# TimeEscaper/distributed_eigenspaces

Measured on AMD Instinct MI355X. Metric: samples/sec ingested + time-to-eigenspace (d=8192,k=64) at 1/8 GPU; sinθ error, higher is better.
Workload: dtype f32

## Files before the change

distributed_eigenspaces_amd/csrc/capi.hip:

```cpp
#include <stdarg.h>
#include <stdio.h>
#include <string.h>

#include <atomic>
#include <vector>

#include "deig_internal.hpp"

namespace deig {

static thread_local char g_err[1024] = "";

const char* last_error() { return g_err; }

void set_error(const char* fmt, ...) {
  va_list ap;
  va_start(ap, fmt);
  vsnprintf(g_err, sizeof(g_err), fmt, ap);
  va_end(ap);
}

int fail(int code, const char* fmt, ...) {
  va_list ap;
  va_start(ap, fmt);
// ... 10 lines not shown
    return 256;
  }
  int v = cache[dev].load(std::memory_order_relaxed);
  if (!v) {
    if (hipDeviceGetAttribute(&v, hipDeviceAttributeMultiprocessorCount, dev) != hipSuccess ||
        v <= 0) {
      (void)hipGetLastError();
      v = 256;
    }
    cache[dev].store(v, std::memory_order_relaxed);
  }
  return v;
}

}

using namespace deig;

extern "C" {

int deig_version(void) { return 0x000600; }

void deig_shutdown(void) {
  if (status_pool_empty()) return;
  (void)hipDeviceSynchronize();
  status_pool_drain();
  (void)hipGetLastError();
}

const char* deig_last_error(void) { return g_err; }

void deig_solver_opts_init(deig_solver_opts* o) {
  if (!o) return;
  memset(o, 0, sizeof(*o));
  o->size = (int)sizeof(deig_solver_opts);
  o->sweep_algo = DEIG_SWEEP_AUTO;
  o->rr_every = 0;
  o->chebyshev = 1;
  o->cheb_above = -1.f;
  o->deflate = 1;
  o->deflate_early = 1;
  o->jacobi_early_sweeps = -1;
  o->jacobi_early_above = -1.f;
  o->fast_until = 1e-3f;
  o->round_until = 1e-4f;
  o->debug = 0;
  o->half_until = 1e-2f;
}

// ... 46 lines not shown
  if (algo != DEIG_SYRK_AUTO) return algo;
  return n >= DEIG_SYRK_SPLIT_MIN_ROWS ? DEIG_SYRK_SPLIT3 : DEIG_SYRK_FP32;
}

size_t deig_syrk_workspace_ex(int64_t n, int64_t d, int algo) {
  algo = syrk_resolve(n, algo & ~DEIG_SYRK_ACCUMULATE);
  if (algo == DEIG_SYRK_FP32) return syrk_workspace_bytes(n, d);
  if (algo == DEIG_SYRK_SPLIT3) return syrk_split_workspace_bytes(n, d);
  return 0;
}

int deig_syrk_f32_ex(const float* X, int64_t n, int64_t d, int64_t ldx, float alpha, float* S,
                     int64_t lds, int algo, void* ws, size_t ws_bytes, void* stream) {
  g_err[0] = 0;
  const bool acc = (algo & DEIG_SYRK_ACCUMULATE) != 0;
  algo = syrk_resolve(n, algo & ~DEIG_SYRK_ACCUMULATE);
  if (acc && algo != DEIG_SYRK_SPLIT3)
    return fail(DEIG_EINVAL, "syrk: DEIG_SYRK_ACCUMULATE needs the split3 algorithm");
  if (algo == DEIG_SYRK_FP32)
    return syrk_launch(X, n, d, ldx, alpha, S, lds, ws, ws_bytes, (hipStream_t)stream);
  if (algo == DEIG_SYRK_SPLIT3)
    return syrk_split_launch(X, n, d, ldx, alpha, S, lds, ws, ws_bytes, (hipStream_t)stream, acc);
  return fail(DEIG_EINVAL, "syrk: unknown algorithm %d", algo);
}

size_t deig_syrk_workspace(int64_t n, int64_t d) {
  return deig_syrk_workspace_ex(n, d, DEIG_SYRK_DEFAULT);
}

int deig_syrk_f32(const float* X, int64_t n, int64_t d, int64_t ldx, float alpha, float* S,
                  int64_t lds, void* ws, size_t ws_bytes, void* stream) {
  return deig_syrk_f32_ex(X, n, d, ldx, alpha, S, lds, DEIG_SYRK_DEFAULT, ws, ws_bytes, stream);
}

size_t deig_syrk_bf16_workspace(int64_t n, int64_t d) { return syrk_bf16_workspace_bytes(n, d); }

int deig_syrk_bf16(const void* X, int64_t n, int64_t d, int64_t ldx, float alpha, float* S,
                   int64_t lds, int flags, void* ws, size_t ws_bytes, void* stream) {
  g_err[0] = 0;
  return syrk_bf16_launch(X, n, d, ldx, alpha, S, lds, flags, ws, ws_bytes, (hipStream_t)stream);
}

size_t deig_syrk_shift_workspace(int64_t n, int64_t d, int xtype) {
  return syrk_shift_workspace_bytes(n, d, xtype);
}

// ... 465 lines not shown
```

distributed_eigenspaces_amd/csrc/deig_internal.hpp:

```cpp
#pragma once

#include <hip/hip_runtime.h>
#include <stdint.h>
#include <stddef.h>

#include "../../include/deig.h"

namespace deig {

typedef float f32x16 __attribute__((ext_vector_type(16)));
typedef float f32x4 __attribute__((ext_vector_type(4)));
typedef float f32x2 __attribute__((ext_vector_type(2)));
typedef double f64x2 __attribute__((ext_vector_type(2)));
typedef __attribute__((address_space(3))) void lds_void;

void set_error(const char* fmt, ...);
int fail(int code, const char* fmt, ...);
const char* last_error();

#define DEIG_HIP_CHECK(expr)                                                          \
  do {                                                                                \
    hipError_t e__ = (expr);                                                          \
    if (e__ != hipSuccess)                                                            \
      return ::deig::fail(DEIG_EHIP, "%s:%d %s: %s", __FILE__, __LINE__, #expr,       \
// ... 30 lines not shown

struct Carve {
  char* base;
  size_t cap;
  size_t off = 0;
  Carve(void* b, size_t c) : base(static_cast<char*>(b)), cap(c) {}
  template <class T>
  T* take(size_t count) {
    off = align_up(off, 256);
    T* p = reinterpret_cast<T*>(base ? base + off : nullptr);
    off += count * sizeof(T);
    return p;
  }
  bool ok() const { return off <= cap; }
};

size_t syrk_workspace_bytes(int64_t n, int64_t d);
int syrk_launch(const float* X, int64_t n, int64_t d, int64_t ldx, float alpha, float* S,
                int64_t lds, void* ws, size_t ws_bytes, hipStream_t stream);
size_t syrk_split_workspace_bytes(int64_t n, int64_t d);
int syrk_split_launch(const float* X, int64_t n, int64_t d, int64_t ldx, float alpha, float* S,
                      int64_t lds, void* ws, size_t ws_bytes, hipStream_t stream,
                      bool accumulate = false);

size_t syrk_bf16_workspace_bytes(int64_t n, int64_t d);
int syrk_bf16_launch(const void* X, int64_t n, int64_t d, int64_t ldx, float alpha, float* S,
                     int64_t lds, int flags, void* ws, size_t ws_bytes, hipStream_t stream);

size_t syrk_shift_workspace_bytes(int64_t n, int64_t d, int xtype);
int syrk_shift_launch(const void* X, int xtype, int64_t n, int64_t d, int64_t ldx, double alpha,
                      double* S64, int64_t lds64, float* S, int64_t lds, void* ws, size_t ws_bytes,
                      hipStream_t stream);

size_t syrk_centered_workspace_bytes(int64_t n, int64_t d, int xtype);
int syrk_centered_launch(const void* X, int xtype, int64_t n, int64_t d, int64_t ldx,
                         const double* center, double alpha, double* S64, int64_t lds64, float* S,
                         int64_t lds, double* mean_out, void* ws, size_t ws_bytes,
                         hipStream_t stream);
size_t colsum_workspace_bytes(int64_t n, int64_t d);
int colsum_launch(const void* X, int xtype, int64_t n, int64_t d, int64_t ldx, double* sums,
                  void* ws, size_t ws_bytes, hipStream_t stream);

size_t syrk_u8_workspace_bytes(int64_t n, int64_t d, int mode);
int syrk_u8_launch(const uint8_t* X, int64_t n, int64_t d, int64_t ldx, int mode, double alpha,
                   float* S, int64_t lds, double* S64, int64_t lds64, void* ws, size_t ws_bytes,
                   hipStream_t stream);
// ... 205 lines not shown
```

distributed_eigenspaces_amd/csrc/lds_dma.hpp:

```cpp
#pragma once

#include "deig_internal.hpp"

namespace deig {

typedef int i32x4 __attribute__((ext_vector_type(4)));

__device__ __forceinline__ i32x4 make_rsrc(const void* base, uint32_t nrec) {
  const uint64_t a = reinterpret_cast<uint64_t>(base);
  i32x4 r;
  r[0] = (int)(uint32_t)a;
  r[1] = (int)((uint32_t)(a >> 32) & 0xffffu);
  r[2] = (int)nrec;
  r[3] = 0x00020000;
  return r;
}

__device__ __forceinline__ void dma16(i32x4 rsrc, int voff, const void* lds_dst) {
  const unsigned m0v = (unsigned)(uintptr_t)(lds_void*)lds_dst;
  asm volatile("s_mov_b32 m0, %2\n\tbuffer_load_dwordx4 %0, %1, 0 offen lds"
               :
               : "v"(voff), "s"(rsrc), "s"(m0v)
               : "memory", "m0");
}

template <int N>
__device__ __forceinline__ void wait_vm() {
  asm volatile("s_waitcnt vmcnt(%0)" ::"n"(N) : "memory");
}

}
```

distributed_eigenspaces_amd/csrc/syrk_split.hip:

```cpp
#include <cmath>
#include <cstdlib>

#include "bf16_split.hpp"
#include "deig_internal.hpp"
#include "lds_dma.hpp"

namespace deig {
namespace {

constexpr int BT = 256;
constexpr int ROWS_PAD = 32;
constexpr int NTHR = 512;
constexpr int SLICE_B = BT * 16;
constexpr int SLAB = BT * BT;
constexpr int SPLIT_YB = 256;
constexpr int SUPER_H = 8, SUPER_W = 4;
constexpr int BLOCK_B = 8 * SLICE_B;
constexpr size_t DEFAULT_CHUNK_BYTES = size_t(64) << 30;

struct SSched {
  unsigned char* XP;
  float* S;
  float* part;
  float* accs;
  const int* order;
  int64_t lds, dp;
  int64_t NK;
  int nseg;
  int d, nt, T, G, q, R;
  float alpha;
  int beta;
  int flush_kt;
  unsigned* pace;
  int pace_kt;
  const float* X;
  int64_t ldx, nrows;
  float* corr;
};

constexpr int kChipPaceEvery = 2;
#ifdef DEIG_AB_SYRK_FLUSH_STAGGER
// ... 56 lines not shown
  const int items = s.R * s.nseg;
  return L < items ? (items - 1 - L) / s.G + 1 : 0;
}

__device__ __forceinline__ void rem_item(const SSched& s, int L, int u, int& tile, int& slot, int& sg) {
  const int i = L + u * s.G;
  sg = i / s.R;
  const int r = i - sg * s.R;
  tile = s.q * s.G + r;
  slot = sg * s.R + r;
}

struct WorkItem {
  int tile, slot, seg;
  int64_t k0, k1;
  bool partial;
  PaceSeq pc;
};

template <bool HALF>
__device__ __forceinline__ WorkItem work_item(const SSched& s, int L, int w) {
  WorkItem it{0, 0, 0, 0, s.NK, w >= s.q, PaceSeq{0, 0u, 0u}};
  const unsigned nx = xcd_blocks(s);
  const unsigned P = s.pace_kt > 0 ? (unsigned)(s.NK / s.pace_kt) : 0u;
  if (!it.partial) {
    it.tile = w * s.G + L;
    it.pc = PaceSeq{(int)P, (unsigned)w * P * nx, nx};
    if (HALF) {
      it.pc.g = true;
      it.pc.gbase = (unsigned)w * (P / kChipPaceEvery) * (unsigned)s.G;
      it.pc.gmult = (unsigned)s.G;
    }
    return it;
  }
  const int u = w - s.q;
  rem_item(s, L, u, it.tile, it.slot, it.seg);
  it.k0 = __builtin_amdgcn_readfirstlane((int)(s.NK * it.seg / s.nseg));
  it.k1 = __builtin_amdgcn_readfirstlane((int)(s.NK * (it.seg + 1) / s.nseg));
  const int Pm = (HALF && s.pace_kt > 0 && s.nseg > 0) ? (int)(s.NK / s.nseg / s.pace_kt) : 0;
  if (Pm > 0) {
    const int items = s.R * s.nseg;
    unsigned before = 0;
    unsigned gb = (unsigned)s.q * (P / kChipPaceEvery) * (unsigned)s.G;
    for (int v = 0; v < u; ++v) {
      before += (unsigned)rem_active(s, L, v);
      gb += (unsigned)min(s.G, items - v * s.G) * (unsigned)(Pm / kChipPaceEvery);
    }
    it.pc = PaceSeq{Pm, (unsigned)s.q * P * nx + before * (unsigned)Pm, (unsigned)rem_active(s, L, u)};
    it.pc.g = true;
    it.pc.gbase = gb;
    it.pc.gmult = (unsigned)min(s.G, items - u * s.G);
  }
  return it;
}

constexpr int PANEL_B = 8 * SLICE_B;
constexpr int BUF_B = 2 * PANEL_B;

constexpr int OCT_B = 2 * SLICE_B;

__device__ __forceinline__ void stage_x(const SSched& s, int64_t kt, int f0, unsigned char* buf,
                                        int wave, int voff) {
  const int64_t row0 = kt * 32 + 8 * (wave & 3);
  int64_t rv = s.nrows - row0;
// ... 170 lines not shown
  }
  if (!diag) {
#pragma unroll
    for (int u = 0; u < 4; ++u) s.S[(int64_t)(ib + u) * s.lds + j] = v[u];
    const f32x4 w = {v[0], v[1], v[2], v[3]};
    *reinterpret_cast<f32x4*>(s.S + (int64_t)j * s.lds + ib) = w;
  } else {
#pragma unroll
    for (int u = 0; u < 4; ++u)
      if (ib + u >= j) {
        s.S[(int64_t)(ib + u) * s.lds + j] = v[u];
        s.S[(int64_t)j * s.lds + ib + u] = v[u];
      }
  }
}

struct TileCtx {
  int lane, wave, wi, wj;
  int ti, tj, i0, j0;
  bool diag;
  float* slab;
};

__device__ __forceinline__ TileCtx tile_ctx(const SSched& s, const WorkItem& it) {
  TileCtx c;
  c.lane = threadIdx.x & 63;
  c.wave = __builtin_amdgcn_readfirstlane(threadIdx.x >> 6);
  c.wi = c.wave >> 2;
  c.wj = c.wave & 3;
  const int tt = __builtin_amdgcn_readfirstlane(s.order[it.tile]);
  c.ti = tt & 0xffff;
  c.tj = tt >> 16;
  c.i0 = c.ti * BT;
  c.j0 = c.tj * BT;
  c.diag = (c.ti == c.tj);
  c.slab = it.partial ? s.part + (int64_t)it.slot * SLAB : s.accs + (int64_t)blockIdx.x * SLAB;
  return c;
}

template <bool IDLE = false>
__device__ __forceinline__ void finish_tile(const SSched& s, const TileCtx c, Acc& acc, bool flushed,
                                            bool partial) {
  if constexpr (!IDLE)
    if (flushed) unflush(c.slab, acc, c.wave, c.lane);
  if (partial) {
#pragma unroll
    for (int q = 0; q < NQUAD; ++q)
      *slab_at(c.slab, c.wave, q, c.lane) = f32x4{acc.at(q, 0), acc.at(q, 1), acc.at(q, 2), acc.at(q, 3)};
    return;
  }
  if constexpr (IDLE) return;
#pragma unroll
  for (int q = 0; q < NQUAD; ++q) {
    const float a[4] = {acc.at(q, 0), acc.at(q, 1), acc.at(q, 2), acc.at(q, 3)};
    store4(s, c.i0 + 128 * c.wi + Acc::qrow(q, c.lane), c.j0 + 64 * c.wj + Acc::qcol(q, c.lane), c.diag, a);
  }
}

template <bool SQ>
__device__ __forceinline__ void segment(const SSched& s, unsigned char* lds, const WorkItem& it) {
  const TileCtx tc = tile_ctx(s, it);
  const int lane = tc.lane, wave = tc.wave, wi = tc.wi, wj = tc.wj;
  const int64_t k0 = it.k0;
  float* const slab = tc.slab;
  const int fx0 = (wave >= 4 && !tc.diag) ? tc.j0 : tc.i0;
  const int fv = s.d - fx0;
  const int xvoff = 4 * lane < fv ? lane * 16 : (1 << 30);
  float sq[4] = {0.f, 0.f, 0.f, 0.f};

  Acc acc;
  acc.zero();
  bool flushed = false;
  const int64_t nkt = it.k1 - k0;
  if (nkt > 0) {
    wait_vm<0>();
    __syncthreads();
    stage_x(s, k0, fx0, lds, wave, xvoff);
    wait_vm<0>();
    const int64_t rv0 = s.nrows - (k0 * 32 + 8 * (wave & 3));
    convert_x<SQ>(lds, wave, lane, rv0 < 0 ? 0 : rv0 > 8 ? 8 : (int)rv0, fv, sq);
    int cur = 0, nxt = 1, since = 0;
    PaceState pace(it.pc);
    for (int64_t t = 0; t < nkt; ++t) {
      pace_point(s, it.pc, pace);
// ... 14 lines not shown
        flushed = true;
        since = 0;
      }
      cur = cur + 1 == 2 ? 0 : cur + 1;
      nxt = nxt + 1 == 2 ? 0 : nxt + 1;
    }
  }
  if (SQ) {
    float* c = s.corr + (int64_t)(it.seg * 4 + wave) * s.dp + tc.i0;
#pragma unroll
    for (int h = 0; h < 2; ++h)
      *reinterpret_cast<f32x2*>(c + 128 * h + 2 * lane) = f32x2{sq[2 * h], sq[2 * h + 1]};
  }
  finish_tile(s, tc, acc, flushed, it.partial);
}

constexpr int kDwOff = -1, kDwDiag = -2;
constexpr bool dw_skip(int dw, int mb, int nb) { return dw >= 0 && 16 * mb + 15 < dw + 16 * nb; }
constexpr bool dw_row(int dw, int mb) { return !dw_skip(dw, mb, 0); }
constexpr bool dw_col(int dw, int nb) { return !dw_skip(dw, 7, nb); }
constexpr bool dw_idle(int dw) { return !dw_row(dw, 7); }

template <int DW>
__device__ __forceinline__ void segment_h(const SSched& s, unsigned char* lds, const WorkItem& it) {
  constexpr bool idle = dw_idle(DW);
  constexpr bool dgb = DW != kDwOff;
  constexpr int QB = 8 * 1024;
  constexpr int BOFF = 4 * QB;
  const TileCtx tc = tile_ctx(s, it);
  const int lane = tc.lane, wave = tc.wave, wi = tc.wi, wj = tc.wj, ti = tc.ti, tj = tc.tj;
  const bool lag = wave >= 4;
  const int64_t k0 = it.k0;
  float* const slab = tc.slab;
  Acc acc;
  acc.zero();
  bool flushed = false;
  const int64_t nkt = it.k1 - k0;
  auto bar = [&]() {
    __builtin_amdgcn_sched_barrier(0);
    __builtin_amdgcn_s_barrier();
    __builtin_amdgcn_sched_barrier(0);
    asm volatile("" ::: "memory");
  };
  const int a_off = ti * BLOCK_B + wave * SLICE_B + ((lane >> 5) * 128 + (lane & 31)) * 16;
  const int b_off = tj * BLOCK_B + wave * SLICE_B + lane * 16;
  const uint32_t nrec = (uint32_t)(s.nt * BLOCK_B);
  auto ring_rsrc = [&](int64_t kt) {
    return make_rsrc(s.XP + kt * (int64_t)s.nt * BLOCK_B, nrec);
  };
  auto issue_a = [&](int64_t kt, int q, unsigned char* buf) {
    const i32x4 r = ring_rsrc(kt);
    int o = a_off + q * 512;
    asm volatile("" : "+v"(o));
    dma16(r, o, buf + q * QB + wave * 1024);
  };
  auto issue_b = [&](int64_t kt, unsigned char* buf, int p0, int p1) {
    const i32x4 r = ring_rsrc(kt);
    int o = b_off;
    asm volatile("" : "+v"(o));
#pragma unroll
    for (int p = 0; p < 4; ++p)
      if (p >= p0 && p < p1) dma16(r, o + p * 1024, buf + BOFF + wave * SLICE_B + p * 1024);
  };
  if (nkt > 0) {
    wait_vm<0>();
    __syncthreads();
    if constexpr (!dgb) issue_b(k0, lds, 0, 4);
#pragma unroll
    for (int q = 0; q < 4; ++q) issue_a(k0, q, lds);
    if (nkt > 1) {
      if constexpr (!dgb) issue_b(k0 + 1, lds + BUF_B, 0, 2);
      issue_a(k0 + 1, 0, lds + BUF_B);
      issue_a(k0 + 1, 1, lds + BUF_B);
      wait_vm<dgb ? 2 : 4>();
    } else {
      wait_vm<0>();
    }
    asm volatile("s_waitcnt lgkmcnt(0)" ::: "memory");
    bar();
    if (lag) bar();
    const int c = lane & 15, g4 = lane >> 4;
    const int xcd = blockIdx.x & 7;
    int since = kFlushStaggerDiv > 0 ? xcd * (s.flush_kt / kFlushStaggerDiv) : 0;
    PaceState pace(it.pc);
    bf16x8 bhi[4], blo[4];
// ... 61 lines not shown
        asm volatile("s_waitcnt lgkmcnt(0)" ::: "memory");
        bar();
#pragma unroll
        for (int m = 0; m < 4; ++m) {
          const int mb = 4 * h + m;
#pragma unroll
          for (int nb = 0; nb < 4; ++nb)
            if (!dw_skip(DW, mb, nb))
              acc.a[mb][nb] = __builtin_amdgcn_mfma_f32_16x16x32_bf16(ahi[m], bhi[nb], acc.a[mb][nb], 0, 0, 0);
#pragma unroll
          for (int nb = 0; nb < 4; ++nb)
            if (!dw_skip(DW, mb, nb))
              acc.a[mb][nb] = __builtin_amdgcn_mfma_f32_16x16x32_bf16(ahi[m], blo[nb], acc.a[mb][nb], 0, 0, 0);
#pragma unroll
          for (int nb = 0; nb < 4; ++nb)
            if (!dw_skip(DW, mb, nb))
              acc.a[mb][nb] = __builtin_amdgcn_mfma_f32_16x16x32_bf16(alo[m], bhi[nb], acc.a[mb][nb], 0, 0, 0);
        }
        bar();
      }
    }
    if (!lag) bar();
  }
  finish_tile<idle>(s, tc, acc, flushed, it.partial);
}

__global__ __launch_bounds__(NTHR) void syrks_h_kernel(SSched s) {
  __shared__ __attribute__((aligned(16))) unsigned char lds[2 * BUF_B];
  const int L = xcd_logical(blockIdx.x, s.G);
  const int nwork = s.q + rem_rounds(s, L);
  for (int w = 0; w < nwork; ++w) {
    const WorkItem it = work_item<true>(s, L, w);
    const int tt = __builtin_amdgcn_readfirstlane(s.order[it.tile]);
    const int wv = __builtin_amdgcn_readfirstlane(threadIdx.x >> 6);
    const bool dg = (tt & 0xffff) == (tt >> 16);
    const int dw = 64 * (wv & 3) - 128 * (wv >> 2);
    if (dg && dw == 0)
      segment_h<0>(s, lds, it);
    else if (dg && dw == 64)
      segment_h<64>(s, lds, it);
    else if (dg && dw >= 128)
      segment_h<128>(s, lds, it);
    else if (dg)
      segment_h<kDwDiag>(s, lds, it);
    else
      segment_h<kDwOff>(s, lds, it);
  }
}

__global__ __launch_bounds__(NTHR) void syrks_kernel(SSched s) {
  __shared__ __attribute__((aligned(16))) unsigned char lds[2 * BUF_B];
  const int L = xcd_logical(blockIdx.x, s.G);
  const int nwork = s.q + rem_rounds(s, L);
  for (int w = 0; w < nwork; ++w) {
    const WorkItem it = work_item<false>(s, L, w);
    const int tt = __builtin_amdgcn_readfirstlane(s.order[it.tile]);
    if ((tt & 0xffff) == (tt >> 16) && (threadIdx.x >> 6) < 4)
      segment<true>(s, lds, it);
    else
      segment<false>(s, lds, it);
  }
}

__global__ __launch_bounds__(256) void syrks_reduce_kernel(SSched s) {
  const int r = blockIdx.x;
  const int f = blockIdx.y * 256 + threadIdx.x;
  const int lane = f & 63, q = (f >> 6) & (NQUAD - 1), wave = f >> 11;
  const int wi = wave >> 2, wj = wave & 3;
  const int tt = s.order[s.q * s.G + r];
// ... 37 lines not shown
#pragma unroll
      for (int p = 0; p < 4; ++p) {
        const uint32_t h0 = bf16_rne(v[q][2 * p]), h1 = bf16_rne(v[q][2 * p + 1]);
        const float r0 = v[q][2 * p] - __uint_as_float(h0 << 16);
        const float r1 = v[q][2 * p + 1] - __uint_as_float(h1 << 16);
        const uint32_t l0 = bf16_rne(r0), l1 = bf16_rne(r1);
        const float lf0 = __uint_as_float(l0 << 16), lf1 = __uint_as_float(l1 << 16);
        sq[q] += lf0 * lf0 + lf1 * lf1;
        hv[p] = h0 | (h1 << 16);
        lv[p] = l0 | (l1 << 16);
      }
      const int64_t f = fb + lane + 64 * q;
      unsigned char* dst = XP + ((o >> 2) * (dp / BT) + (f / BT)) * BLOCK_B +
                           ((o & 3) * 2) * SLICE_B + (f % BT) * 16;
      __builtin_nontemporal_store(hv, reinterpret_cast<u32x4*>(dst));
      __builtin_nontemporal_store(lv, reinterpret_cast<u32x4*>(dst + SLICE_B));
    }
  }
#pragma unroll
  for (int q = 0; q < 4; ++q) red[w][lane + 64 * q] = sq[q];
  __syncthreads();
  const int t = threadIdx.x;
  corr[(int64_t)blockIdx.y * dp + fb + t] = red[0][t] + red[1][t] + red[2][t] + red[3][t];
}

__global__ __launch_bounds__(256) void diag_corr_kernel(const float* __restrict__ corr, int yb,
                                                        int64_t dp, int d, float alpha, float* S,
                                                        int64_t lds) {
  __shared__ float part[4][64];
  const int t = threadIdx.x & 63, sl = threadIdx.x >> 6;
  const int i = blockIdx.x * 64 + t;
  float c = 0.f;
  if (i < d) {
#pragma unroll 8
    for (int y = sl; y < yb; y += 4) c += corr[(int64_t)y * dp + i];
  }
  part[sl][t] = c;
  __syncthreads();
  if (sl == 0 && i < d) S[(int64_t)i * lds + i] += alpha * (((part[0][t] + part[1][t]) + part[2][t]) + part[3][t]);
}

__global__ __launch_bounds__(256) void tile_order_kernel(int nt, int* order) {
  const int nsc = (nt + SUPER_W - 1) / SUPER_W;
  const int u = blockIdx.x * 256 + threadIdx.x;
  const int R0 = (u / nsc) * SUPER_H, C0 = (u % nsc) * SUPER_W;
  if (R0 >= nt) return;
// ... 27 lines not shown
  while ((a + 1) * (a + 1) <= u) ++a;
  const int item = u - a * a;
  int* grp = order + 32 * u;
  if (item == 0) {
    int i = 0;
    for (int ti = 8 * a; ti < 8 * a + 8; ++ti)
      for (int tj = 8 * a; tj <= ti; ++tj) {
        const int v = ti | (tj << 16);
        if (i < 32) grp[i] = v;
        else order[32 * m * m + 4 * a + (i - 32)] = v;
        ++i;
      }
  } else {
    const int b = (item - 1) >> 1, h = (item - 1) & 1;
    int i = 0;
    for (int ti = 8 * a; ti < 8 * a + 8; ++ti)
      for (int tj = 8 * b + 4 * h; tj < 8 * b + 4 * h + 4; ++tj) grp[i++] = ti | (tj << 16);
  }
}

struct Layout {
  int64_t dp, nt, T, G, q, R, nseg, yb_max, chunk_rows;
  size_t off_order, off_pace, off_accs, off_part, off_corr, off_xp, total;
};

Layout make_layout(int64_t d, int G, int64_t chunk_rows) {
  Layout L;
  L.dp = cdiv(d, BT) * BT;
  L.nt = L.dp / BT;
  L.T = L.nt * (L.nt + 1) / 2;
  L.G = G;
  L.q = L.T / G;
  L.R = L.T % G;
  L.nseg = remainder_segments(L.R, G);
  L.yb_max = SPLIT_YB;
  L.chunk_rows = chunk_rows;
  size_t off = 0;
  L.off_order = off;
  off = align_up(off + sizeof(int) * L.T, 256);
  L.off_pace = off;
  off += 16 * 128;
  L.off_accs = off;
  off += sizeof(float) * (size_t)G * SLAB;
  L.off_part = off;
  off += sizeof(float) * (size_t)(L.R * L.nseg) * SLAB;
  L.off_corr = off;
  off = align_up(off + sizeof(float) * (size_t)L.yb_max * L.dp, 256);
  L.off_xp = off;
  off += (size_t)chunk_rows * L.dp * 4;
  L.total = off;
  return L;
}

int64_t default_chunk_rows(int64_t n, int64_t d) {
  const int64_t dp = cdiv(d, BT) * BT;
  const int64_t n32 = cdiv(n, ROWS_PAD) * ROWS_PAD;
  int64_t cap = (int64_t)(DEFAULT_CHUNK_BYTES / (size_t)(dp * 4)) / ROWS_PAD * ROWS_PAD;
  if (cap < ROWS_PAD) cap = ROWS_PAD;
  return n32 < cap ? n32 : cap;
}

constexpr int64_t kFusedMaxD = 2048;

int flush_ktiles(int64_t n) {
#ifdef DEIG_AB_SYRK_FLUSH_ROWS
  int64_t flush_rows = DEIG_AB_SYRK_FLUSH_ROWS;
  (void)n;
#else
  int64_t flush_rows = 4096;
  while (flush_rows < 16384 && (flush_rows * 2) * (flush_rows * 2) <= 128 * n) flush_rows *= 2;
#endif
  return flush_rows < ROWS_PAD ? 1 : (int)(flush_rows / ROWS_PAD);
// ... 30 lines not shown
  s.ldx = ldx;
  s.nrows = n;
  s.corr = reinterpret_cast<float*>(base + L.off_corr);
  return s;
}

int run_pass(const SSched& s, const Layout& L, int64_t yb, hipStream_t stream) {
  if (s.pace_kt > 0) DEIG_HIP_CHECK(hipMemsetAsync(s.pace, 0, 9 * 128, stream));
  if (s.d <= kFusedMaxD)
    hipLaunchKernelGGL(syrks_kernel, dim3((unsigned)L.G), dim3(NTHR), 0, stream, s);
  else
    hipLaunchKernelGGL(syrks_h_kernel, dim3((unsigned)L.G), dim3(NTHR), 0, stream, s);
  DEIG_HIP_CHECK(hipGetLastError());
  if (s.R > 0) {
    hipLaunchKernelGGL(syrks_reduce_kernel, dim3(s.R, SLAB / 4 / 256), dim3(256), 0, stream, s);
    DEIG_HIP_CHECK(hipGetLastError());
  }
  hipLaunchKernelGGL(diag_corr_kernel, dim3((unsigned)cdiv(s.d, 64)), dim3(256), 0, stream, s.corr,
                     (int)yb, L.dp, s.d, s.alpha, s.S, s.lds);
  DEIG_HIP_CHECK(hipGetLastError());
  return DEIG_OK;
}

}

int syrk_cus() {
#ifdef DEIG_AB_SYRK_G
  return DEIG_AB_SYRK_G;
#else
  return num_cus();
#endif
}

size_t syrk_split_workspace_bytes(int64_t n, int64_t d) {
  if (n < 1 || d < 1) return 0;
  return make_layout(d, syrk_cus(), d <= kFusedMaxD ? 0 : default_chunk_rows(n, d)).total;
}

int syrk_split_launch(const float* X, int64_t n, int64_t d, int64_t ldx, float alpha, float* S,
                      int64_t lds, void* ws, size_t ws_bytes, hipStream_t stream, bool accumulate) {
  DEIG_REQUIRE(n >= 1, "syrk: n must be >= 1 (got %lld)", (long long)n);
  DEIG_REQUIRE(d >= 1 && d % 4 == 0, "syrk: d must be a positive multiple of 4 (got %lld)",
               (long long)d);
  DEIG_REQUIRE(d <= (1 << 16) - BT, "syrk: d too large (%lld)", (long long)d);
  DEIG_REQUIRE(ldx >= d && ldx % 4 == 0, "syrk: ldx must be >= d and a multiple of 4");
  DEIG_REQUIRE(lds >= d && lds % 4 == 0, "syrk: lds must be >= d and a multiple of 4");
  DEIG_REQUIRE(X && S && aligned16(X) && aligned16(S), "syrk: X and S must be 16-byte aligned");
  const int G = syrk_cus();
  const bool fused = d <= kFusedMaxD;
  const Layout L0 = make_layout(d, G, 0);
  const size_t ws_min = L0.total + (fused ? 0 : (size_t)ROWS_PAD * L0.dp * 4);
  if (!ws || ws_bytes < ws_min)
    return fail(DEIG_EWORKSPACE, "syrk: workspace %zu bytes < minimum %zu", ws_bytes, ws_min);
  int64_t chunk = (int64_t)((ws_bytes - L0.total) / (size_t)(L0.dp * 4)) / ROWS_PAD * ROWS_PAD;
  const int64_t n32 = cdiv(n, ROWS_PAD) * ROWS_PAD;
  if (chunk > n32) chunk = n32;
  const Layout L = make_layout(d, G, fused ? 0 : chunk);
  char* base = static_cast<char*>(ws);
  SSched s = make_sched(L, base, X, n, d, ldx, alpha, S, lds);
  if (G == 256 && s.nt % 8 == 0)
    hipLaunchKernelGGL(tile_order_compact_kernel, dim3((unsigned)cdiv((s.nt / 8) * (s.nt / 8), 256)), dim3(256), 0,
                       stream, s.nt, reinterpret_cast<int*>(base + L.off_order));
  else
    hipLaunchKernelGGL(tile_order_kernel,
                       dim3((unsigned)cdiv(cdiv(s.nt, SUPER_H) * cdiv(s.nt, SUPER_W), 256)), dim3(256), 0, stream,
                       s.nt, reinterpret_cast<int*>(base + L.off_order));
  DEIG_HIP_CHECK(hipGetLastError());
  if (fused) {
    DEIG_REQUIRE(ldx <= (int64_t(1) << 25), "syrk: ldx > 2^25 is not supported for d <= 2048");
    const int64_t yb = 4 * (L.nseg > 1 ? L.nseg : 1);
    DEIG_REQUIRE(yb <= L.yb_max, "syrk: %lld lo^2 partial rows exceed the workspace's %lld",
                 (long long)yb, (long long)L.yb_max);
    DEIG_HIP_CHECK(hipMemsetAsync(s.corr, 0, sizeof(float) * (size_t)(yb * L.dp), stream));
    s.NK = cdiv(n, ROWS_PAD);
    s.beta = accumulate ? 1 : 0;
    return run_pass(s, L, yb, stream);
  }
  for (int64_t r0 = 0, c = 0; r0 < n; r0 += chunk, ++c) {
    const int64_t rows = (n - r0) < chunk ? (n - r0) : chunk;
    const int64_t nk = cdiv(rows, ROWS_PAD);
    const int64_t noct = nk * (ROWS_PAD / 8);
    int64_t yb = cdiv(noct, 4);
    if (yb > L.yb_max) yb = L.yb_max;
    hipLaunchKernelGGL(split_kernel, dim3((unsigned)(L.dp / 256), (unsigned)yb), dim3(256), 0,
                       stream, X + r0 * ldx, rows, ldx, (int)d, L.dp, noct, s.XP, s.corr);
    DEIG_HIP_CHECK(hipGetLastError());
    s.NK = nk;
    s.beta = (c > 0 || accumulate) ? 1 : 0;
    if (int rc = run_pass(s, L, yb, stream)) return rc;
  }
  return DEIG_OK;
}

}
```

Baseline: 7.425 million.

## Pipeline chunked split3 SYRK by overlapping next-chunk splitting on a side stream

After: 7.405 million. About the same (-0.3%).

```diff
diff --git a/distributed_eigenspaces_amd/csrc/capi.hip b/distributed_eigenspaces_amd/csrc/capi.hip
--- a/distributed_eigenspaces_amd/csrc/capi.hip
+++ b/distributed_eigenspaces_amd/csrc/capi.hip
@@ -56,9 +56,10 @@
 int deig_version(void) { return 0x000600; }
 
 void deig_shutdown(void) {
-  if (status_pool_empty()) return;
+  if (status_pool_empty() && syrk_split_idle()) return;
   (void)hipDeviceSynchronize();
   status_pool_drain();
+  syrk_split_release();
   (void)hipGetLastError();
 }
 
@@ -151,6 +152,14 @@
   if (algo == DEIG_SYRK_SPLIT3)
     return syrk_split_launch(X, n, d, ldx, alpha, S, lds, ws, ws_bytes, (hipStream_t)stream, acc);
   return fail(DEIG_EINVAL, "syrk: unknown algorithm %d", algo);
+}
+
+int64_t deig_internal_syrk_split_chunks(const float* X, int64_t n, int64_t d, int64_t ldx, float alpha,
+                                        float* S, int64_t lds, int64_t chunk_rows, int pipelined,
+                                        int accumulate, void* ws, size_t ws_bytes, void* stream) {
+  g_err[0] = 0;
+  return syrk_split_chunks(X, n, d, ldx, alpha, S, lds, chunk_rows, pipelined != 0, ws, ws_bytes,
+                           (hipStream_t)stream, accumulate != 0);
 }
 
 size_t deig_syrk_workspace(int64_t n, int64_t d) {
diff --git a/distributed_eigenspaces_amd/csrc/deig_internal.hpp b/distributed_eigenspaces_amd/csrc/deig_internal.hpp
--- a/distributed_eigenspaces_amd/csrc/deig_internal.hpp
+++ b/distributed_eigenspaces_amd/csrc/deig_internal.hpp
@@ -76,6 +76,12 @@
 int syrk_split_launch(const float* X, int64_t n, int64_t d, int64_t ldx, float alpha, float* S,
                       int64_t lds, void* ws, size_t ws_bytes, hipStream_t stream,
                       bool accumulate = false);
+
+bool syrk_split_idle();
+void syrk_split_release();
+int64_t syrk_split_chunks(const float* X, int64_t n, int64_t d, int64_t ldx, float alpha, float* S,
+                          int64_t lds, int64_t chunk_rows, bool pipelined, void* ws, size_t ws_bytes,
+                          hipStream_t stream, bool accumulate);
 
 size_t syrk_bf16_workspace_bytes(int64_t n, int64_t d);
 int syrk_bf16_launch(const void* X, int64_t n, int64_t d, int64_t ldx, float alpha, float* S,
diff --git a/distributed_eigenspaces_amd/csrc/lds_dma.hpp b/distributed_eigenspaces_amd/csrc/lds_dma.hpp
--- a/distributed_eigenspaces_amd/csrc/lds_dma.hpp
+++ b/distributed_eigenspaces_amd/csrc/lds_dma.hpp
@@ -24,6 +24,16 @@
                : "memory", "m0");
 }
 
+template <int OFF>
+__device__ __forceinline__ void dma16(i32x4 rsrc, int voff, const void* lds_dst) {
+  static_assert(OFF >= 0 && OFF < 4096, "buffer instruction offsets are 12 bits");
+  const unsigned m0v = (unsigned)(uintptr_t)(lds_void*)lds_dst - (unsigned)OFF;
+  asm volatile("s_mov_b32 m0, %2\n\tbuffer_load_dwordx4 %0, %1, 0 offen offset:%3 lds"
+               :
+               : "v"(voff), "s"(rsrc), "s"(m0v), "n"(OFF)
+               : "memory", "m0");
+}
+
 template <int N>
 __device__ __forceinline__ void wait_vm() {
   asm volatile("s_waitcnt vmcnt(%0)" ::"n"(N) : "memory");
diff --git a/distributed_eigenspaces_amd/csrc/syrk_split.hip b/distributed_eigenspaces_amd/csrc/syrk_split.hip
--- a/distributed_eigenspaces_amd/csrc/syrk_split.hip
+++ b/distributed_eigenspaces_amd/csrc/syrk_split.hip
@@ -1,5 +1,6 @@
 #include <cmath>
 #include <cstdlib>
+#include <mutex>
 
 #include "bf16_split.hpp"
 #include "deig_internal.hpp"
@@ -17,6 +18,17 @@
 constexpr int SUPER_H = 8, SUPER_W = 4;
 constexpr int BLOCK_B = 8 * SLICE_B;
 constexpr size_t DEFAULT_CHUNK_BYTES = size_t(64) << 30;
+constexpr int kSyrkVgprs = 240;
+constexpr int kSplitVgprs = 32;
+static_assert(2 * kSyrkVgprs + kSplitVgprs <= 512 && kSyrkVgprs % 8 == 0 && kSplitVgprs % 8 == 0,
+              "a SYRK block and a splitter workgroup must fit one CU's register files");
+constexpr int64_t kPipeMinRows = 65536;
+constexpr int kPipeChunks = 4;
+#ifdef DEIG_AB_SYRK_PIPELINE
+constexpr bool kPipeline = DEIG_AB_SYRK_PIPELINE != 0;
+#else
+constexpr bool kPipeline = true;
+#endif
 
 struct SSched {
   unsigned char* XP;
@@ -119,7 +131,9 @@
 __device__ __forceinline__ WorkItem work_item(const SSched& s, int L, int w) {
   WorkItem it{0, 0, 0, 0, s.NK, w >= s.q, PaceSeq{0, 0u, 0u}};
   const unsigned nx = xcd_blocks(s);
-  const unsigned P = s.pace_kt > 0 ? (unsigned)(s.NK / s.pace_kt) : 0u;
+  int nseg = s.nseg, pace_kt = s.pace_kt;
+  if constexpr (HALF) asm volatile("" : "+s"(nseg), "+s"(pace_kt));
+  const unsigned P = pace_kt > 0 ? (unsigned)(s.NK / pace_kt) : 0u;
   if (!it.partial) {
     it.tile = w * s.G + L;
     it.pc = PaceSeq{(int)P, (unsigned)w * P * nx, nx};
@@ -132,11 +146,11 @@
   }
   const int u = w - s.q;
   rem_item(s, L, u, it.tile, it.slot, it.seg);
-  it.k0 = __builtin_amdgcn_readfirstlane((int)(s.NK * it.seg / s.nseg));
-  it.k1 = __builtin_amdgcn_readfirstlane((int)(s.NK * (it.seg + 1) / s.nseg));
-  const int Pm = (HALF && s.pace_kt > 0 && s.nseg > 0) ? (int)(s.NK / s.nseg / s.pace_kt) : 0;
+  it.k0 = __builtin_amdgcn_readfirstlane((int)(s.NK * it.seg / nseg));
+  it.k1 = __builtin_amdgcn_readfirstlane((int)(s.NK * (it.seg + 1) / nseg));
+  const int Pm = (HALF && pace_kt > 0 && nseg > 0) ? (int)(s.NK / nseg / pace_kt) : 0;
   if (Pm > 0) {
-    const int items = s.R * s.nseg;
+    const int items = s.R * nseg;
     unsigned before = 0;
     unsigned gb = (unsigned)s.q * (P / kChipPaceEvery) * (unsigned)s.G;
     for (int v = 0; v < u; ++v) {
@@ -353,13 +367,12 @@
   float* slab;
 };
 
-__device__ __forceinline__ TileCtx tile_ctx(const SSched& s, const WorkItem& it) {
+__device__ __forceinline__ TileCtx tile_ctx(const SSched& s, const WorkItem& it, unsigned tid, int tt) {
   TileCtx c;
-  c.lane = threadIdx.x & 63;
-  c.wave = __builtin_amdgcn_readfirstlane(threadIdx.x >> 6);
+  c.lane = tid & 63;
+  c.wave = __builtin_amdgcn_readfirstlane(tid >> 6);
   c.wi = c.wave >> 2;
   c.wj = c.wave & 3;
-  const int tt = __builtin_amdgcn_readfirstlane(s.order[it.tile]);
   c.ti = tt & 0xffff;
   c.tj = tt >> 16;
   c.i0 = c.ti * BT;
@@ -390,7 +403,7 @@
 
 template <bool SQ>
 __device__ __forceinline__ void segment(const SSched& s, unsigned char* lds, const WorkItem& it) {
-  const TileCtx tc = tile_ctx(s, it);
+  const TileCtx tc = tile_ctx(s, it, threadIdx.x, __builtin_amdgcn_readfirstlane(s.order[it.tile]));
   const int lane = tc.lane, wave = tc.wave, wi = tc.wi, wj = tc.wj;
   const int64_t k0 = it.k0;
   float* const slab = tc.slab;
@@ -451,12 +464,12 @@
 constexpr bool dw_idle(int dw) { return !dw_row(dw, 7); }
 
 template <int DW>
-__device__ __forceinline__ void segment_h(const SSched& s, unsigned char* lds, const WorkItem& it) {
+__device__ __forceinline__ void segment_h(const SSched& s, unsigned char* lds, const WorkItem& it, unsigned tid, int tt) {
   constexpr bool idle = dw_idle(DW);
   constexpr bool dgb = DW != kDwOff;
   constexpr int QB = 8 * 1024;
   constexpr int BOFF = 4 * QB;
-  const TileCtx tc = tile_ctx(s, it);
+  const TileCtx tc = tile_ctx(s, it, tid, tt);
   const int lane = tc.lane, wave = tc.wave, wi = tc.wi, wj = tc.wj, ti = tc.ti, tj = tc.tj;
   const bool lag = wave >= 4;
   const int64_t k0 = it.k0;
@@ -479,17 +492,20 @@
   };
   auto issue_a = [&](int64_t kt, int q, unsigned char* buf) {
     const i32x4 r = ring_rsrc(kt);
-    int o = a_off + q * 512;
-    asm volatile("" : "+v"(o));
-    dma16(r, o, buf + q * QB + wave * 1024);
+    switch (q) {
+      case 0: dma16<0>(r, a_off, buf + wave * 1024); break;
+      case 1: dma16<512>(r, a_off, buf + QB + wave * 1024); break;
+      case 2: dma16<1024>(r, a_off, buf + 2 * QB + wave * 1024); break;
+      default: dma16<1536>(r, a_off, buf + 3 * QB + wave * 1024); break;
+    }
   };
   auto issue_b = [&](int64_t kt, unsigned char* buf, int p0, int p1) {
     const i32x4 r = ring_rsrc(kt);
-    int o = b_off;
-    asm volatile("" : "+v"(o));
-#pragma unroll
-    for (int p = 0; p < 4; ++p)
-      if (p >= p0 && p < p1) dma16(r, o + p * 1024, buf + BOFF + wave * SLICE_B + p * 1024);
+    unsigned char* dst = buf + BOFF + wave * SLICE_B;
+    if (0 >= p0 && 0 < p1) dma16<0>(r, b_off, dst);
+    if (1 >= p0 && 1 < p1) dma16<1024>(r, b_off, dst + 1024);
+    if (2 >= p0 && 2 < p1) dma16<2048>(r, b_off, dst + 2048);
+    if (3 >= p0 && 3 < p1) dma16<3072>(r, b_off, dst + 3072);
   };
   if (nkt > 0) {
     wait_vm<0>();
@@ -597,29 +613,32 @@
     }
     if (!lag) bar();
   }
-  finish_tile<idle>(s, tc, acc, flushed, it.partial);
-}
-
-__global__ __launch_bounds__(NTHR) void syrks_h_kernel(SSched s) {
+  asm volatile("" : "+v"(tid));
+  finish_tile<idle>(s, tile_ctx(s, it, tid, tt), acc, flushed, it.partial);
+}
+
+__global__ __launch_bounds__(NTHR) __attribute__((amdgpu_num_vgpr(kSyrkVgprs / 2))) void syrks_h_kernel(SSched s) {
   __shared__ __attribute__((aligned(16))) unsigned char lds[2 * BUF_B];
   const int L = xcd_logical(blockIdx.x, s.G);
   const int nwork = s.q + rem_rounds(s, L);
   for (int w = 0; w < nwork; ++w) {
     const WorkItem it = work_item<true>(s, L, w);
     const int tt = __builtin_amdgcn_readfirstlane(s.order[it.tile]);
-    const int wv = __builtin_amdgcn_readfirstlane(threadIdx.x >> 6);
+    unsigned tid = threadIdx.x;
+    asm volatile("" : "+v"(tid));
+    const int wv = __builtin_amdgcn_readfirstlane(tid >> 6);
     const bool dg = (tt & 0xffff) == (tt >> 16);
     const int dw = 64 * (wv & 3) - 128 * (wv >> 2);
     if (dg && dw == 0)
-      segment_h<0>(s, lds, it);
+      segment_h<0>(s, lds, it, tid, tt);
     else if (dg && dw == 64)
-      segment_h<64>(s, lds, it);
+      segment_h<64>(s, lds, it, tid, tt);
     else if (dg && dw >= 128)
-      segment_h<128>(s, lds, it);
+      segment_h<128>(s, lds, it, tid, tt);
     else if (dg)
-      segment_h<kDwDiag>(s, lds, it);
+      segment_h<kDwDiag>(s, lds, it, tid, tt);
     else
-      segment_h<kDwOff>(s, lds, it);
+      segment_h<kDwOff>(s, lds, it, tid, tt);
   }
 }
 
@@ -703,6 +722,55 @@
   __syncthreads();
   const int t = threadIdx.x;
   corr[(int64_t)blockIdx.y * dp + fb + t] = red[0][t] + red[1][t] + red[2][t] + red[3][t];
+}
+
+constexpr int kSplitNextLds = 20 * 1024;
+__global__ __launch_bounds__(256) __attribute__((amdgpu_num_vgpr(kSplitVgprs / 2)))
+void split_next_kernel(const float* __restrict__ X, int64_t n, int64_t ldx, int d, int64_t dp,
+                       int64_t noct, int yb, unsigned char* __restrict__ XP,
+                       float* __restrict__ corr) {
+  __shared__ float red[kSplitNextLds / 4];
+  const int lane = threadIdx.x & 63, w = __builtin_amdgcn_readfirstlane(threadIdx.x >> 6);
+  const int ng = (int)(dp / 64);
+  const int units = yb * ng;
+  const int nt = (int)(dp / BT);
+  for (int u = blockIdx.x; u < units; u += gridDim.x) {
+    const int y = u / ng, g = u - y * ng;
+    const int f = g * 64 + lane;
+    const int ld_off = f * 4;
+    const int st_off = (f / BT) * BLOCK_B + (f % BT) * 16;
+    float sq = 0.f;
+    for (int64_t o = (int64_t)y * 4 + w; o < noct; o += (int64_t)yb * 4) {
+      float v[8];
+#pragma unroll
+      for (int r = 0; r < 8; ++r) {
+        const int64_t row = o * 8 + r;
+        const __amdgpu_buffer_rsrc_t rs = __builtin_amdgcn_make_buffer_rsrc(
+            const_cast<float*>(X + row * ldx), (short)0, row < n ? d * 4 : 0, 0x00020000);
+        v[r] = __builtin_bit_cast(float, __builtin_amdgcn_raw_buffer_load_b32(rs, ld_off, 0, 2));
+      }
+      u32x4 hv, lv;
+#pragma unroll
+      for (int p = 0; p < 4; ++p) {
+        const uint32_t hh = cvt2(v[2 * p], v[2 * p + 1]);
+        const uint32_t ll = cvt2(v[2 * p] - lo_f(hh), v[2 * p + 1] - hi_f(hh));
+        const float lf0 = lo_f(ll), lf1 = hi_f(ll);
+        sq += lf0 * lf0 + lf1 * lf1;
+        hv[p] = hh;
+        lv[p] = ll;
+      }
+      const int sl = ((int)(o & 3) * 2) * SLICE_B;
+      const __amdgpu_buffer_rsrc_t ws = __builtin_amdgcn_make_buffer_rsrc(
+          XP + (o >> 2) * (int64_t)nt * BLOCK_B + sl, (short)0, nt * BLOCK_B - sl, 0x00020000);
+      __builtin_amdgcn_raw_buffer_store_b128(hv, ws, st_off, 0, 2);
+      __builtin_amdgcn_raw_buffer_store_b128(lv, ws, st_off + SLICE_B, 0, 2);
+    }
+    red[w * 64 + lane] = sq;
+    __syncthreads();
+    if (w == 0)
+      corr[(int64_t)y * dp + f] = red[lane] + red[64 + lane] + red[128 + lane] + red[192 + lane];
+    __syncthreads();
+  }
 }
 
 __global__ __launch_bounds__(256) void diag_corr_kernel(const float* __restrict__ corr, int yb,
@@ -776,9 +844,10 @@
 struct Layout {
   int64_t dp, nt, T, G, q, R, nseg, yb_max, chunk_rows;
   size_t off_order, off_pace, off_accs, off_part, off_corr, off_xp, total;
+  size_t corr_bytes, xp_bytes;
 };
 
-Layout make_layout(int64_t d, int G, int64_t chunk_rows) {
+Layout make_layout(int64_t d, int G, int64_t chunk_rows, int nbuf = 1) {
   Layout L;
   L.dp = cdiv(d, BT) * BT;
   L.nt = L.dp / BT;
@@ -799,9 +868,11 @@
   L.off_part = off;
   off += sizeof(float) * (size_t)(L.R * L.nseg) * SLAB;
   L.off_corr = off;
-  off = align_up(off + sizeof(float) * (size_t)L.yb_max * L.dp, 256);
+  L.corr_bytes = align_up(sizeof(float) * (size_t)L.yb_max * L.dp, 256);
+  off = align_up(off, 256) + (size_t)nbuf * L.corr_bytes;
   L.off_xp = off;
-  off += (size_t)chunk_rows * L.dp * 4;
+  L.xp_bytes = (size_t)chunk_rows * L.dp * 4;
+  off += (size_t)nbuf * L.xp_bytes;
   L.total = off;
   return L;
 }
@@ -878,6 +949,52 @@
   return DEIG_OK;
 }
 
+struct Pipe {
+  hipStream_t side = nullptr;
+  hipEvent_t entry = nullptr, split[2] = {nullptr, nullptr}, pass[2] = {nullptr, nullptr};
+};
+constexpr int kMaxDevices = 64;
+std::mutex g_pipe_mu;
+Pipe g_pipe[kMaxDevices];
+bool g_pipe_live = false;
+
+int pipe_get(Pipe** out) {
+  int dev = 0;
+  DEIG_HIP_CHECK(hipGetDevice(&dev));
+  DEIG_REQUIRE(dev >= 0 && dev < kMaxDevices, "syrk: device %d out of range", dev);
+  Pipe& p = g_pipe[dev];
+  if (!p.side) {
+    int least = 0, greatest = 0;
+    DEIG_HIP_CHECK(hipDeviceGetStreamPriorityRange(&least, &greatest));
+    hipEvent_t* ev[5] = {&p.entry, &p.split[0], &p.split[1], &p.pass[0], &p.pass[1]};
+    for (hipEvent_t* e : ev)
+      if (!*e) DEIG_HIP_CHECK(hipEventCreateWithFlags(e, hipEventDisableTiming));
+    g_pipe_live = true;
+    DEIG_HIP_CHECK(hipStreamCreateWithPriority(&p.side, hipStreamNonBlocking, least));
+  }
+  *out = &p;
+  return DEIG_OK;
+}
+
+}
+
+bool syrk_split_idle() {
+  std::lock_guard<std::mutex> lock(g_pipe_mu);
+  return !g_pipe_live;
+}
+
+void syrk_split_release() {
+  std::lock_guard<std::mutex> lock(g_pipe_mu);
+  for (Pipe& p : g_pipe) {
+    if (p.side) (void)hipStreamDestroy(p.side);
+    hipEvent_t* ev[5] = {&p.entry, &p.split[0], &p.split[1], &p.pass[0], &p.pass[1]};
+    for (hipEvent_t* e : ev) {
+      if (*e) (void)hipEventDestroy(*e);
+      *e = nullptr;
+    }
+    p.side = nullptr;
+  }
+  g_pipe_live = false;
 }
 
 int syrk_cus() {
@@ -893,8 +1010,76 @@
   return make_layout(d, syrk_cus(), d <= kFusedMaxD ? 0 : default_chunk_rows(n, d)).total;
 }
 
-int syrk_split_launch(const float* X, int64_t n, int64_t d, int64_t ldx, float alpha, float* S,
-                      int64_t lds, void* ws, size_t ws_bytes, hipStream_t stream, bool accumulate) {
+namespace {
+
+int64_t pipe_chunk_rows(int64_t n32, int64_t dp, size_t avail, size_t corr_bytes) {
+  if (!kPipeline || avail <= corr_bytes) return 0;
+  if ((int64_t)(avail / (size_t)(dp * 4)) >= n32) return 0;
+  int64_t rows = (int64_t)((avail - corr_bytes) / 2 / (size_t)(dp * 4)) / ROWS_PAD * ROWS_PAD;
+  const int64_t want = cdiv(cdiv(n32, kPipeChunks), ROWS_PAD) * ROWS_PAD;
+  if (rows > want) rows = want;
+  return rows >= kPipeMinRows && rows < n32 ? rows : 0;
+}
+
+int run_chunks(SSched s, const Layout& L, char* base, const float* X, int64_t n, int64_t ldx,
+               int64_t chunk, bool pipelined, bool accumulate, hipStream_t stream) {
+  std::unique_lock<std::mutex> lock(g_pipe_mu, std::defer_lock);
+  Pipe* pp = nullptr;
+  if (pipelined) {
+    lock.lock();
+    if (int rc = pipe_get(&pp)) return rc;
+  }
+  auto xp_of = [&](int64_t c) {
+    return reinterpret_cast<unsigned char*>(base + L.off_xp + (pipelined ? (size_t)(c & 1) * L.xp_bytes : 0));
+  };
+  auto corr_of = [&](int64_t c) {
+    return reinterpret_cast<float*>(base + L.off_corr + (pipelined ? (size_t)(c & 1) * L.corr_bytes : 0));
+  };
+  struct Chunk {
+    int64_t rows, nk, noct, yb;
+  };
+  auto chunk_of = [&](int64_t r0) {
+    Chunk k;
+    k.rows = (n - r0) < chunk ? (n - r0) : chunk;
+    k.nk = cdiv(k.rows, ROWS_PAD);
+    k.noct = k.nk * (ROWS_PAD / 8);
+    k.yb = cdiv(k.noct, 4);
+    if (k.yb > L.yb_max) k.yb = L.yb_max;
+    return k;
+  };
+  for (int64_t r0 = 0, c = 0; r0 < n; r0 += chunk, ++c) {
+    const Chunk k = chunk_of(r0);
+    s.XP = xp_of(c);
+    s.corr = corr_of(c);
+    if (c == 0 || !pipelined) {
+      hipLaunchKernelGGL(split_kernel, dim3((unsigned)(L.dp / 256), (unsigned)k.yb), dim3(256), 0,
+                         stream, X + r0 * ldx, k.rows, ldx, s.d, L.dp, k.noct, s.XP, s.corr);
+      DEIG_HIP_CHECK(hipGetLastError());
+      if (pipelined) {
+        DEIG_HIP_CHECK(hipEventRecord(pp->entry, stream));
+        DEIG_HIP_CHECK(hipStreamWaitEvent(pp->side, pp->entry, 0));
+      }
+    } else {
+      DEIG_HIP_CHECK(hipStreamWaitEvent(stream, pp->split[c & 1], 0));
+    }
+    s.NK = k.nk;
+    s.beta = (c > 0 || accumulate) ? 1 : 0;
+    if (int rc = run_pass(s, L, k.yb, stream)) return rc;
+    if (pipelined && r0 + chunk < n) {
+      const Chunk nx = chunk_of(r0 + chunk);
+      DEIG_HIP_CHECK(hipEventRecord(pp->pass[c & 1], stream));
+      if (c > 0) DEIG_HIP_CHECK(hipStreamWaitEvent(pp->side, pp->pass[(c - 1) & 1], 0));
+      hipLaunchKernelGGL(split_next_kernel, dim3((unsigned)L.G), dim3(256), 0, pp->side,
+                         X + (r0 + chunk) * ldx, nx.rows, ldx, s.d, L.dp, nx.noct, (int)nx.yb,
+                         xp_of(c + 1), corr_of(c + 1));
+      DEIG_HIP_CHECK(hipGetLastError());
+      DEIG_HIP_CHECK(hipEventRecord(pp->split[(c + 1) & 1], pp->side));
+    }
+  }
+  return DEIG_OK;
+}
+
+int check_args(const float* X, int64_t n, int64_t d, int64_t ldx, float* S, int64_t lds) {
   DEIG_REQUIRE(n >= 1, "syrk: n must be >= 1 (got %lld)", (long long)n);
   DEIG_REQUIRE(d >= 1 && d % 4 == 0, "syrk: d must be a positive multiple of 4 (got %lld)",
                (long long)d);
@@ -902,6 +1087,24 @@
   DEIG_REQUIRE(ldx >= d && ldx % 4 == 0, "syrk: ldx must be >= d and a multiple of 4");
   DEIG_REQUIRE(lds >= d && lds % 4 == 0, "syrk: lds must be >= d and a multiple of 4");
   DEIG_REQUIRE(X && S && aligned16(X) && aligned16(S), "syrk: X and S must be 16-byte aligned");
+  return DEIG_OK;
+}
+
+void launch_tile_order(const SSched& s, int G, int* order, hipStream_t stream) {
+  if (G == 256 && s.nt % 8 == 0)
+    hipLaunchKernelGGL(tile_order_compact_kernel, dim3((unsigned)cdiv((s.nt / 8) * (s.nt / 8), 256)), dim3(256), 0,
+                       stream, s.nt, order);
+  else
+    hipLaunchKernelGGL(tile_order_kernel,
+                       dim3((unsigned)cdiv(cdiv(s.nt, SUPER_H) * cdiv(s.nt, SUPER_W), 256)), dim3(256), 0, stream,
+                       s.nt, order);
+}
+
+}
+
+int syrk_split_launch(const float* X, int64_t n, int64_t d, int64_t ldx, float alpha, float* S,
+                      int64_t lds, void* ws, size_t ws_bytes, hipStream_t stream, bool accumulate) {
+  if (int rc = check_args(X, n, d, ldx, S, lds)) return rc;
   const int G = syrk_cus();
   const bool fused = d <= kFusedMaxD;
   const Layout L0 = make_layout(d, G, 0);
@@ -911,16 +1114,12 @@
   int64_t chunk = (int64_t)((ws_bytes - L0.total) / (size_t)(L0.dp * 4)) / ROWS_PAD * ROWS_PAD;
   const int64_t n32 = cdiv(n, ROWS_PAD) * ROWS_PAD;
   if (chunk > n32) chunk = n32;
-  const Layout L = make_layout(d, G, fused ? 0 : chunk);
+  const int64_t pchunk = fused ? 0 : pipe_chunk_rows(n32, L0.dp, ws_bytes - L0.total, L0.corr_bytes);
+  if (pchunk > 0) chunk = pchunk;
+  const Layout L = make_layout(d, G, fused ? 0 : chunk, pchunk > 0 ? 2 : 1);
   char* base = static_cast<char*>(ws);
   SSched s = make_sched(L, base, X, n, d, ldx, alpha, S, lds);
-  if (G == 256 && s.nt % 8 == 0)
-    hipLaunchKernelGGL(tile_order_compact_kernel, dim3((unsigned)cdiv((s.nt / 8) * (s.nt / 8), 256)), dim3(256), 0,
-                       stream, s.nt, reinterpret_cast<int*>(base + L.off_order));
-  else
-    hipLaunchKernelGGL(tile_order_kernel,
-                       dim3((unsigned)cdiv(cdiv(s.nt, SUPER_H) * cdiv(s.nt, SUPER_W), 256)), dim3(256), 0, stream,
-                       s.nt, reinterpret_cast<int*>(base + L.off_order));
+  launch_tile_order(s, G, reinterpret_cast<int*>(base + L.off_order), stream);
   DEIG_HIP_CHECK(hipGetLastError());
   if (fused) {
     DEIG_REQUIRE(ldx <= (int64_t(1) << 25), "syrk: ldx > 2^25 is not supported for d <= 2048");
@@ -932,20 +1131,26 @@
     s.beta = accumulate ? 1 : 0;
     return run_pass(s, L, yb, stream);
   }
-  for (int64_t r0 = 0, c = 0; r0 < n; r0 += chunk, ++c) {
-    const int64_t rows = (n - r0) < chunk ? (n - r0) : chunk;
-    const int64_t nk = cdiv(rows, ROWS_PAD);
-    const int64_t noct = nk * (ROWS_PAD / 8);
-    int64_t yb = cdiv(noct, 4);
-    if (yb > L.yb_max) yb = L.yb_max;
-    hipLaunchKernelGGL(split_kernel, dim3((unsigned)(L.dp / 256), (unsigned)yb), dim3(256), 0,
-                       stream, X + r0 * ldx, rows, ldx, (int)d, L.dp, noct, s.XP, s.corr);
-    DEIG_HIP_CHECK(hipGetLastError());
-    s.NK = nk;
-    s.beta = (c > 0 || accumulate) ? 1 : 0;
-    if (int rc = run_pass(s, L, yb, stream)) return rc;
-  }
-  return DEIG_OK;
-}
-
-}
+  return run_chunks(s, L, base, X, n, ldx, chunk, pchunk > 0, accumulate, stream);
+}
+
+int64_t syrk_split_chunks(const float* X, int64_t n, int64_t d, int64_t ldx, float alpha, float* S,
+                          int64_t lds, int64_t chunk_rows, bool pipelined, void* ws, size_t ws_bytes,
+                          hipStream_t stream, bool accumulate) {
+  if (d <= kFusedMaxD || chunk_rows < ROWS_PAD || chunk_rows % ROWS_PAD != 0)
+    return fail(DEIG_EINVAL, "syrk chunks: need d > %lld and chunk_rows a positive multiple of %d",
+                (long long)kFusedMaxD, ROWS_PAD);
+  const int G = syrk_cus();
+  const Layout L = make_layout(d, G, chunk_rows, pipelined ? 2 : 1);
+  if (!ws) return (int64_t)L.total;
+  if (int rc = check_args(X, n, d, ldx, S, lds)) return rc;
+  if (ws_bytes < L.total)
+    return fail(DEIG_EWORKSPACE, "syrk chunks: workspace %zu bytes < %zu", ws_bytes, L.total);
+  char* base = static_cast<char*>(ws);
+  SSched s = make_sched(L, base, X, n, d, ldx, alpha, S, lds);
+  launch_tile_order(s, G, reinterpret_cast<int*>(base + L.off_order), stream);
+  DEIG_HIP_CHECK(hipGetLastError());
+  return run_chunks(s, L, base, X, n, ldx, chunk_rows, pipelined, accumulate, stream);
+}
+
+}
```
